# martinmodrak/math

Measured on AMD Instinct MI355X. Metric: gradient evals/sec (fp64), GP-marginal log-density N=4096, higher is better.
Workload: dtype f64; 1 GPU; gp_marginal_gradient; N=4096, kernel=exp_quad, parallelism=replicas1

## Files before the change

include/smg_hip.h:

```cpp
#ifndef SMG_HIP_H
#define SMG_HIP_H

#include <stddef.h>

#ifdef __cplusplus
extern "C" {
#endif

enum smg_status_code {
  SMG_OK = 0,
  SMG_ERR_HIP = 1,
  SMG_ERR_NOT_PD = 2,
  SMG_ERR_NOT_SYMMETRIC = 4,
  SMG_ERR_NONFINITE = 8,
  SMG_ERR_ARG = 16,
  SMG_ERR_OOM = 32,
  SMG_ERR_NOT_POSITIVE = 64,
  SMG_ERR_SYNC = 128
};

typedef struct smg_ctx smg_ctx;

int smg_device_count(int* n_host);
int smg_ctx_create(int device, size_t initial_arena_bytes, smg_ctx** out_host);
// ... 10 lines not shown
void* smg_host_scratch(smg_ctx* ctx, size_t bytes);
void* smg_pinned_io(smg_ctx* ctx, size_t bytes);
void* smg_pinned_result(smg_ctx* ctx, size_t bytes);
int smg_publish_to_host(smg_ctx* ctx, const double* src, long long n, double* dst);
int smg_gather_scalars(smg_ctx* ctx, const double* const* src, int n, double* dst, int* status_out);

int smg_memcpy_h2d(smg_ctx* ctx, void* dst, const void* src_host, size_t bytes);
int smg_memcpy_d2h(smg_ctx* ctx, void* dst_host, const void* src, size_t bytes);
int smg_memcpy_d2d(smg_ctx* ctx, void* dst, const void* src, size_t bytes);
int smg_memset(smg_ctx* ctx, void* dst, int value, size_t bytes);
int smg_memset_async(smg_ctx* ctx, void* dst, size_t bytes);
int smg_join_async(smg_ctx* ctx);
int smg_sync(smg_ctx* ctx);
int smg_sync_all(smg_ctx* ctx);
int smg_marker_record(smg_ctx* ctx, int slot);
int smg_marker_wait(smg_ctx* ctx, int slot);
int smg_status(smg_ctx* ctx, int* status_host);
int smg_status_armed(smg_ctx* ctx, int* armed);
int smg_status_enqueue(smg_ctx* ctx, int* host_dst);
int smg_status_inject(smg_ctx* ctx, int bits);
int smg_set_inv_block_mode(smg_ctx* ctx, int mode);
int smg_inv_block_fused(smg_ctx* ctx, int n);
int smg_set_gemm_stage_mode(smg_ctx* ctx, int mode);

enum smg_family {
  SMG_FAM_GEMM = 0, SMG_FAM_CHOL_FWD = 1, SMG_FAM_CHOL_REV = 2,
  SMG_FAM_GP = 3, SMG_FAM_MVN = 4, SMG_FAM_TRSV = 5, SMG_FAM_GLM = 6,
  SMG_FAM_ELEMWISE = 7,
  SMG_FAM_PANEL = 8,
  SMG_FAM_COMM = 9,
  SMG_FAM_COUNT = 10
};
int smg_profile_enable(smg_ctx* ctx, int on);
int smg_profile_read(smg_ctx* ctx, int family, double* total_ms_host, long long* count_host);
int smg_profile_flops(smg_ctx* ctx, int family, double* flops_host);

int smg_fill_unif(smg_ctx* ctx, double* out, long long n, unsigned long long seed,
                  double a, double b, double scale);
int smg_fill_bernoulli(smg_ctx* ctx, int* out, long long n, unsigned long long seed, double p);

int smg_gemm(smg_ctx* ctx, int transA, int transB, int uplo, int m, int n, int k,
             double alpha, const double* A, int lda, const double* B, int ldb,
             double beta, double* C, int ldc);
#define SMG_TRI_A_LOWER 1
#define SMG_TRI_A_UPPER 2
#define SMG_TRI_B_LOWER 4
#define SMG_TRI_B_UPPER 8
int smg_gemm_tri(smg_ctx* ctx, int transA, int transB, int uplo, int tri, int m, int n, int k, double alpha,
                 const double* A, int lda, const double* B, int ldb, double beta, double* C, int ldc);
int smg_gemm_bz(smg_ctx* ctx, int transA, int transB, int uplo, int tri, int m, int n, int k, double alpha,
                const double* A, int lda, const double* B, int ldb, double beta, double* C, int ldc, int bz);


int smg_gp_exp_quad_cov_fwd(smg_ctx* ctx, const double* x, int n, double sigma,
                            double l, double* K, int ldk);
int smg_gp_exp_quad_cov_rev(smg_ctx* ctx, const double* x, int n, double sigma,
                            double l, const double* Kadj, int ldka, double* out2);

int smg_gp_exp_quad_cov_nd_fwd(smg_ctx* ctx, const double* x, int D, int n, double sigma,
                               double l, double* K, int ldk);
int smg_gp_exp_quad_cov_nd_rev(smg_ctx* ctx, const double* x, int D, int n, double sigma,
                               double l, const double* Kadj, int ldka, double* out2);

enum smg_gp_family { SMG_GP_EXP_QUAD = 0, SMG_GP_EXPONENTIAL = 1, SMG_GP_MATERN32 = 2, SMG_GP_MATERN52 = 3 };
int smg_gp_cov_fwd(smg_ctx* ctx, int family, const double* x, int D, int n, double sigma, double l,
                   double* K, int ldk);
int smg_gp_cov_rev(smg_ctx* ctx, int family, const double* x, int D, int n, double sigma, double l,
                   const double* Kadj, int ldka, double* out2);

int smg_gp_exp_quad_cov_tangent_fwd(smg_ctx* ctx, const double* x, int n, double sigma,
                                    double l, double dsigma, double dl, double* Kd, int ldk);
int smg_gp_exp_quad_cov_tangent_rev(smg_ctx* ctx, const double* x, int n, double sigma,
                                    double l, double dsigma, double dl, const double* Kdadj,
                                    int ldka, double* out4);
// ... 246 lines not shown
```

math_amd/csrc/chol_mvn.hip:

```cpp
#include "smg_internal.h"
#include "tri_small.h"
#include "gp_family.h"

#include <vector>

namespace {

int inv_t_rec(smg_ctx* ctx, const double* L, int ldl, const double* w512, int n, double* V, int ldv, double* T,
              int lo, int hi, bool pairs) {
  if (hi - lo == SMG_NBR || (pairs && hi - lo == 2 * SMG_NBR)) return SMG_OK;
  const int mid = lo + ((hi - lo) / SMG_NBR / 2) * SMG_NBR;
  int rc = inv_t_rec(ctx, L, ldl, w512, n, V, ldv, T, lo, mid, pairs);
  if (!rc) rc = inv_t_rec(ctx, L, ldl, w512, n, V, ldv, T, mid, hi, pairs);
  if (rc) return rc;
  const int b = mid - lo, a = hi - mid;
  rc = smg_gemm_impl(ctx, 0, 1, 0, b, a, b, 1.0, V + lo + (size_t)lo * ldv, ldv, L + mid + (size_t)lo * ldl, ldl, 0.0,
                     T, n, SMG_TRI_A_UPPER);
  if (rc) return rc;
  return smg_gemm_impl(ctx, 0, 0, 0, b, a, a, -1.0, T, n, V + mid + (size_t)mid * ldv, ldv, 0.0,
                       V + lo + (size_t)mid * ldv, ldv, SMG_TRI_B_UPPER);
}

__global__ __launch_bounds__(256) void k_leaf_transpose(const double* __restrict__ w512, int n, int lo,
                                                       double* __restrict__ V, int ldv) {
// ... 294 lines not shown
  else if (pairs)
    hipLaunchKernelGGL((k_gp_inv_reduce<F, true, true>), dim3(nb), dim3(256), 0, ctx->stream, C, ldc, n, s, k,
                       s_stride, K0, ldk, x, D, cl, s2, part);
  else
    hipLaunchKernelGGL((k_gp_inv_reduce<F, false, true>), dim3(nb), dim3(256), 0, ctx->stream, C, ldc, n, s, k,
                       s_stride, K0, ldk, x, D, cl, s2, part);
  hipLaunchKernelGGL(k_gp_inv_final<F>, dim3(1), dim3(1024), 0, ctx->stream, part, nb, adj, sigma, l, dadj, out2);
  SMG_LAUNCH_CHECK();
  return SMG_OK;
}

}

bool smg_inv_prog_ok(int n) { return n % SMG_NBR == 0 && n >= 2 * SMG_NBR; }

int smg_inv_prog_init(smg_ctx* ctx, int n, double* ws) {
  (void)ctx;
  (void)n;
  (void)ws;
  return SMG_OK;
}

static int prog_acc(smg_ctx* ctx, int ta, int uplo, int m, int nc, int kk, const double* A, int lda,
                    const double* B, int ldb, double* C, int ldc, int bz, bool first) {
  if (first) return smg_gemm_impl(ctx, ta, 0, uplo, m, nc, kk, 1.0, A, lda, B, ldb, 0.0, C, ldc);
  return smg_gemm_bz_impl(ctx, ta, 0, uplo, m, nc, kk, 1.0, A, lda, B, ldb, 1.0, C, ldc, 0, bz);
}

int smg_inv_prog_row(smg_ctx* ctx, const double* L, int ldl, double* aux, int n, double* ws, int k, int part,
                     bool inverses_here) {
  constexpr int P = SMG_NBR;
  const size_t nn = (size_t)n * n;
  double* W = ws;
  double* C = ws + nn;
  double* Y = C + nn;
  double* T = Y + nn;
  const int r0 = k * P, r1 = r0 + P;
  const double* Wkk = aux + (size_t)n * SMG_AUX_W512 + r0;
  int rc;
  switch (part) {
    case 0:
      if (inverses_here) {
        bool wrote = false;
        if ((rc = smg_block_inverses_rows(ctx, L, ldl, aux, n, r0, P, T, W + r0 + (size_t)r0 * n, &wrote)))
          return rc;
        SMG_HIP_TRY(hipEventRecord(ctx->inv_ev_aux, ctx->stream));
        if (wrote) return SMG_OK;
      }
      return smg_copy_impl(ctx, P, P, Wkk, n, W + r0 + (size_t)r0 * n, n, 1.0, 0);
    case 1:
      if (k == 0) return SMG_OK;
      return smg_gemm_impl(ctx, 0, 0, 0, P, r0, P, -1.0, Wkk, n, Y + r0, n, 0.0, W + r0, n, SMG_TRI_A_LOWER);
    case 2:
      return prog_acc(ctx, 1, 1, r1, r1, P, W + r0, n, W + r0, n, C, n, r0, k == 0);
    case 3:
      if (r1 >= n) return SMG_OK;
      return prog_acc(ctx, 0, 0, P, r1, P, L + r1 + (size_t)r0 * ldl, ldl, W + r0, n, Y + r1, n, -r0, k == 0);
    default:
      if (r1 + P >= n) return SMG_OK;
      return prog_acc(ctx, 0, 0, n - r1 - P, r1, P, L + r1 + P + (size_t)r0 * ldl, ldl, W + r0, n, Y + r1 + P, n, -r0,
                      k == 0);
  }
}

double smg_inv_prog_cost(int n, int k, int part, bool inverses_here) {
  constexpr double P = SMG_NBR, rate = 30e6;
  const double r0 = k * P, r1 = r0 + P;
  switch (part) {
    case 0: return inverses_here ? 60.0 : 6.0;
    case 1: return k == 0 ? 0.0 : 6.0 + P * r0 * P / rate;
    case 2: return 6.0 + r1 * r1 * P / rate;
    case 3: return r1 >= n ? 0.0 : 6.0 + 2.0 * P * r1 * P / rate;
    default: return r1 + P >= n ? 0.0 : 6.0 + 2.0 * (n - r1 - P) * r1 * P / rate;
  }
}

extern "C" {

size_t smg_cholesky_mvn_rev_ws_doubles(int n) {
  return n > 0 ? 3 * (size_t)n * n + SMG_NBR / 2 * 256 : 0;
}

int smg_cholesky_mvn_rev(smg_ctx* ctx, const double* L, int ldl, const double* aux, int n, const double* s, int k,
                         long long s_stride, double adj, double* Aadj, int ldaa, double* ws) {
  if (!ctx || n < 0 || k < 1 || (k > 1 && s_stride < n)) return SMG_ERR_ARG;
  if (n == 0) return SMG_OK;
  if (!L || !ws || ldl < n || (Aadj && (!s || ldaa < n))) return SMG_ERR_ARG;
  smg_prof_scope prof(ctx, SMG_FAM_CHOL_REV);
  const size_t nn = (size_t)n * n;
  double* V = ws;
  double* C = ws + nn;
  int rc;
  if (v_by_doubling(n, aux)) {
    if ((rc = form_v(ctx, L, ldl, aux, n, V, C))) return rc;
    rc = smg_gemm_impl(ctx, 0, 1, 1, n, n, n, 1.0, V, n, V, n, 0.0, C, n, SMG_TRI_A_UPPER | SMG_TRI_B_LOWER);
  } else {
// ... 165 lines not shown
```

math_amd/csrc/cholesky.hip:

```cpp
#include <chrono>
#include "smg_internal.h"
#include "tri_small.h"
#include "smg_sync.h"
#include <cstdlib>
#include <vector>

namespace {

__global__ __launch_bounds__(256) void k_check_symmetric(const double* __restrict__ A, int lda,
                                                         int n, int* status) {
  __shared__ double T[64][65];
  int bi, bj;
  {
    const int t = blockIdx.x;
    int r = (int)((sqrt(8.0 * (double)t + 1.0) - 1.0) * 0.5);
    while ((r + 1) * (r + 2) / 2 <= t) ++r;
    while (r * (r + 1) / 2 > t) --r;
    bi = r;
    bj = t - r * (r + 1) / 2;
  }
  const int i0 = 64 * bi, j0 = 64 * bj;
  const int lane = threadIdx.x & 63, w = threadIdx.x >> 6;
  for (int c = w; c < 64; c += 4) {
    const int gr = j0 + lane, gc = i0 + c;
    T[c][lane] = (gr < n && gc < n) ? A[gr + (size_t)gc * lda] : 0.0;
  }
  __syncthreads();
  bool bad = false;
// ... 1621 lines not shown
        smg_on_side on(ctx);
        rc = smg_gemm_impl(ctx, 0, 1, 1, m2, K3 - K2, K - J, -1.0, P2, ldl, P2, ldl, 1.0,
                           L + K2 + (size_t)K2 * ldl, ldl);
      }
      if (rc) return rc;
      F = smg_event(ctx, nev++);
      if (!F) return SMG_ERR_HIP;
      SMG_HIP_TRY(hipEventRecord(F, ctx->side));
      if (K3 < n) {
        const int m3 = n - K3;
        const double* P3 = L + K3 + (size_t)J * ldl;
        smg_on_side on(ctx);
        if ((rc = smg_gemm_impl(ctx, 0, 1, 1, m3, m3, K - J, -1.0, P3, ldl, P3, ldl, 1.0, L + K3 + (size_t)K3 * ldl,
                                ldl)))
          return rc;
      }
    } else if (prog) {
      SMG_HIP_TRY(hipStreamWaitEvent(ctx->side, E, 0));
    }
    if (prog) {
      const double m2 = n - K2, kk = K - J;
      const double slack = 22.0 * (K2 - K) / SMG_NB + 6.0 + (double)(n - K) * (K2 - K) * kk / 30e6 -
                           (K2 < n ? 6.0 + m2 * m2 * kk / 40e6 : 0.0);
      if ((rc = queue_parts(J / NB2, 0.5 * slack))) return rc;
    }
  }
  if (prog) {
    if (int rc0 = queue_parts(rows_prog - 2, -1.0)) return rc0;
  }
  if (mark) {
    const int rc = smg_status_mark_impl(ctx);
    if (rc) return rc;
  }
  if (F) SMG_HIP_TRY(hipStreamWaitEvent(ctx->stream, F, 0));
  int rc;
  if (prog) {
    const int r0 = n - SMG_NBR;
    SMG_HIP_TRY(hipStreamWaitEvent(ctx->stream, ctx->inv_ev_aux, 0));
    bool wkk = false;
    if ((rc = chol_block_inverses(ctx, L, ldl, aux, n, r0, SMG_NBR, nullptr, true, inv_ws + r0 + (size_t)r0 * n,
                                  &wkk)))
      return rc;
    SMG_HIP_TRY(hipEventRecord(ctx->inv_ev_main, ctx->stream));
    const int klast = n / SMG_NBR - 1;
    if (zero_parts) {
      SMG_HIP_TRY(hipStreamWaitEvent(ctx->zero_stream, ctx->inv_ev_main, 0));
      hipStream_t keep = ctx->stream;
// ... 67 lines not shown
```

math_amd/csrc/ctx.hip:

```cpp
#include <cstdio>
#include <cstdlib>
#include <cstring>

#include "smg_internal.h"

namespace {

constexpr size_t kAlign = 256;

__global__ void k_reduce_partials(const double* __restrict__ p, int nparts,
                                  int width, double* out, int accumulate) {
  __shared__ double lds[16];
  const int c = blockIdx.x;
  double s = 0.0;
  for (int i = threadIdx.x; i < nparts; i += blockDim.x) s += p[(size_t)i * width + c];
  s = block_sum(s, lds);
  if (threadIdx.x == 0) out[c] = accumulate ? out[c] + s : s;
}

__global__ __launch_bounds__(256) void k_publish(const double* __restrict__ src, long long n, double* dst,
                                                 long long* done, long long seq) {
  for (long long i = threadIdx.x; i < n; i += blockDim.x)
    __hip_atomic_store(dst + i, src[i], __ATOMIC_RELAXED, __HIP_MEMORY_SCOPE_SYSTEM);
  asm volatile("s_waitcnt vmcnt(0)" ::: "memory");
// ... 209 lines not shown
    return SMG_ERR_HIP;
  }
  if (initial < (size_t)(64u << 20)) initial = (size_t)(64u << 20);
  char* base = nullptr;
  if (hipMalloc(&base, initial) != hipSuccess) {
    hipStreamDestroy(ctx->stream);
    delete ctx;
    return SMG_ERR_OOM;
  }
  ctx->blocks.push_back({base, initial});
  if (hipMalloc(&ctx->status_d, SMG_STATUS_BYTES) != hipSuccess ||
      hipHostMalloc(&ctx->status_h, 256, hipHostMallocDefault) != hipSuccess) {
    delete ctx;
    return SMG_ERR_HIP;
  }
  hipMemset(ctx->status_d, 0, SMG_STATUS_BYTES);
  ctx->flags_d = ctx->status_d + 64;
  ctx->flag_epoch = 0;
  ctx->inv_ctr_d = reinterpret_cast<unsigned*>(ctx->flags_d + 4096);
  ctx->inv_launches = 0;
  ctx->inv_per_cu = ctx->inv_cus = -1;
  ctx->inv_mode = 0;
  ctx->gemm_stage = 0;
  ctx->host_scratch_size = 1u << 20;
  if (hipHostMalloc(&ctx->host_scratch, ctx->host_scratch_size, hipHostMallocDefault) != hipSuccess) {
    delete ctx;
    return SMG_ERR_HIP;
  }
  if (hipHostMalloc(&ctx->done_h, 256, hipHostMallocCoherent | hipHostMallocMapped) != hipSuccess ||
      hipMalloc(&ctx->red_counter_d, 256) != hipSuccess) {
    delete ctx;
    return SMG_ERR_HIP;
  }
  *(volatile long long*)ctx->done_h = 0;
  hipMemset(ctx->red_counter_d, 0, 256);
  hipDeviceSynchronize();
  *out = ctx;
  return SMG_OK;
}

int smg_ctx_destroy(smg_ctx* ctx) {
  if (!ctx) return SMG_OK;
  hipSetDevice(ctx->device);
  hipStreamSynchronize(ctx->stream);
  prof_drain(ctx);
  smg_comm_destroy(ctx);
// ... 350 lines not shown
  if (int rc = smg_marker_event(ctx, slot, &e)) return rc;
  SMG_HIP_TRY(hipEventRecord(e, ctx->stream));
  return SMG_OK;
}

int smg_marker_wait(smg_ctx* ctx, int slot) {
  if (!ctx || slot < 0 || slot >= (int)ctx->marker_ev.size()) return SMG_ERR_ARG;
  SMG_HIP_TRY(hipEventSynchronize(ctx->marker_ev[slot]));
  return SMG_OK;
}

int smg_set_inv_block_mode(smg_ctx* ctx, int mode) {
  if (!ctx || mode < 0 || mode > 1) return SMG_ERR_ARG;
  ctx->inv_mode = mode;
  return SMG_OK;
}

int smg_set_gemm_stage_mode(smg_ctx* ctx, int mode) {
  if (!ctx || mode < 0 || mode > 2) return SMG_ERR_ARG;
  ctx->gemm_stage = mode;
  return SMG_OK;
}

int smg_sync_all(smg_ctx* ctx) {
  if (!ctx) return SMG_ERR_ARG;
  sync_all_streams(ctx);
  SMG_HIP_TRY(hipGetLastError());
  if (ctx->prof_on) prof_drain(ctx);
  return SMG_OK;
}

int smg_sync(smg_ctx* ctx) {
  SMG_HIP_TRY(hipStreamSynchronize(ctx->stream));
  if (ctx->prof_on) prof_drain(ctx);
  return SMG_OK;
}

int smg_status(smg_ctx* ctx, int* status) {
  hipLaunchKernelGGL(k_status_take, dim3(1), dim3(64), 0, ctx->stream, ctx->status_d, ctx->status_h);
  SMG_LAUNCH_CHECK();
  SMG_HIP_TRY(hipStreamSynchronize(ctx->stream));
  if (ctx->prof_on) prof_drain(ctx);
  int s = ctx->status_h[0] | ctx->host_status;
  ctx->host_status = 0;
  ctx->status_armed = 0;
  if (status) *status = s;
// ... 137 lines not shown
```

math_amd/csrc/gemm.hip:

```cpp
#include "smg_internal.h"
#include <cstdio>
#include <cstdlib>
#include <type_traits>

#ifndef SMG_GEMM_TRI128_MIN
#define SMG_GEMM_TRI128_MIN 1024
#endif
#ifndef SMG_GEMM_KS2_MAX
#define SMG_GEMM_KS2_MAX 1536
#endif
#ifndef SMG_GEMM_DMA_BK1
#define SMG_GEMM_DMA_BK1 16
#endif
#ifndef SMG_GEMM_DMA_NB1
#define SMG_GEMM_DMA_NB1 3
#endif
#ifndef SMG_GEMM_DMA_BK2
#define SMG_GEMM_DMA_BK2 32
#endif
#ifndef SMG_GEMM_DMA_NB2
#define SMG_GEMM_DMA_NB2 2
#endif
#ifndef SMG_GEMM_DMA_KS2_MAX
#define SMG_GEMM_DMA_KS2_MAX 512
// ... 122 lines not shown
  tri_decode(t, r, c);
  const int r0 = r / G * G, r1 = min(r0 + G, T), h = r1 - r0;
  int q = t - r0 * (r0 + 1) / 2;
  if (q < r0 * h) {
    bi = r0 + q % h;
    bj = q / h;
    return;
  }
  q -= r0 * h;
  int j = r0;
  while (q >= r1 - j) {
    q -= r1 - j;
    ++j;
  }
  bi = j + q;
  bj = j;
}

template <int BM, int BN, int BK, bool TA, bool TB, int MODE, int KS = 1, int NB = 0>
__global__ __launch_bounds__(256 * KS) void k_gemm(
    int m, int n, int k, double alpha, const double* __restrict__ A, int lda,
    const double* __restrict__ B, int ldb, double beta, double* __restrict__ C,
    int ldc, int tiles_m, int ntiles, int kchunk, double* __restrict__ slab, long long sA,
    long long sB, long long sC, int px, int ntp, int tri, double* __restrict__ C2, int ldc2, int bz) {
  constexpr bool LOWT = MODE == 1 || MODE == 3;
  constexpr bool UPT = MODE == 2;
  constexpr bool TRIC = LOWT || UPT;
  A += blockIdx.y * sA;
  B += blockIdx.y * sB;
  C += blockIdx.y * sC;
  constexpr bool AK = TA;
  constexpr bool BKC = !TB;
  using LA = lds_layout<BM, BK, AK>;
  using LB = lds_layout<BN, BK, BKC>;
  constexpr int NR = BM == 128 ? 1 : (BM == 64 ? SMG_GEMM_NR64 : SMG_GEMM_NR32);
  constexpr int STAGE = LA::size + LB::size;
  constexpr int OPS = (NB ? NB : 2) * STAGE;
  constexpr int ECH = (BM * BN + BN <= OPS) ? BN : 32;
  constexpr int POOL = (OPS > (BM + 1) * ECH) ? OPS : (BM + 1) * ECH;
  __shared__ double pool[POOL];

  int bi, bj, tile, split;
  const bool tri_a_only = !TRIC && (tri & 3) && !(tri & 12);
  const bool tri_b_only = !TRIC && (tri & 12) && !(tri & 3);
  if (px > 0) {
    split = blockIdx.x / ntp;
    const int tb = blockIdx.x - split * ntp;
    const int x = tb & 7, l = tb >> 3, py = 8 / px;
    const int tiles_n = ntiles / tiles_m;
    const int rx = x % px, ry = x / px;
    const int r0 = rx * tiles_m / px, r1 = (rx + 1) * tiles_m / px;
    const int c0 = ry * tiles_n / py, c1 = (ry + 1) * tiles_n / py;
    const int rm = r1 - r0;
    if (rm <= 0 || l >= rm * (c1 - c0)) return;
    tile = (r0 + l % rm) + (c0 + l / rm) * tiles_m;
  } else {
    tile = blockIdx.x % ntiles;
    split = blockIdx.x / ntiles;
  }
  const bool tri_sq = TRIC && m == n && BM == BN;
  if (LOWT && tri_sq) {
    const int T = tiles_m;
    int r, q;
    if (tri == SMG_TRI_B_LOWER) {
      tri_decode(ntiles - 1 - tile, r, q);
      bj = T - 1 - r;
      bi = bj + q;
    } else if (tri == SMG_TRI_B_UPPER || tri == (SMG_TRI_A_LOWER | SMG_TRI_B_UPPER)) {
      tri_decode(tile, r, q);
      bj = T - 1 - r;
      bi = bj + q;
    } else if (tri == (SMG_TRI_A_LOWER | SMG_TRI_B_LOWER)) {
      tri_decode(tile, r, q);
      bj = q;
      bi = q + (T - 1 - r);
    } else if (tri == SMG_TRI_A_LOWER) {
      tri_decode(ntiles - 1 - tile, bi, bj);
    } else if (tri == 0 && ntiles >= 64) {
      const int b = tile, x = b & 7, per = ntiles >> 3, extra = ntiles & 7;
      tri_decode_grouped(x * per + (x < extra ? x : extra) + (b >> 3), tiles_m, bi, bj);
    } else {
      tri_decode(tile, bi, bj);
    }
  } else if (UPT && tri_sq) {
    tri_decode(tile, bj, bi);
  } else if (tri_a_only) {
    const int r = tile / (ntiles / tiles_m);
    bi = (tri & 1) ? tiles_m - 1 - r : r;
    bj = tile % (ntiles / tiles_m);
  } else if (tri_b_only) {
    const int tn = ntiles / tiles_m, c = tile / tiles_m;
    bi = tile % tiles_m;
    bj = (tri & 8) ? tn - 1 - c : c;
  } else {
    bi = tile % tiles_m;
    bj = tile / tiles_m;
  }
  if (LOWT && !tri_sq && bj * BN > bi * BM + BM - 1) return;
  if (UPT && !tri_sq && bi * BM > bj * BN + BN - 1) return;
  const int i0 = bi * BM, j0 = bj * BN;
  int kbeg = split * kchunk;
  int kend = min(k, kbeg + kchunk);
  if (tri) {
    int lo = 0, hi = k;
    if (tri & 1) hi = min(hi, i0 + BM);
    if (tri & 2) lo = max(lo, i0);
    if (tri & 4) lo = max(lo, j0);
    if (tri & 8) hi = min(hi, j0 + BN);
    lo = lo / BK * BK;
    kbeg = max(kbeg, lo);
    kend = min(kend, hi);
    if (kend < kbeg) kend = kbeg;
  }

  constexpr int TM = BM / 32, TN = BN / 32;
  constexpr int NT = 256 * KS;
  const int lane = threadIdx.x & 63, wave = threadIdx.x >> 6;
  const int wr = (wave & 3) >> 1, wc = wave & 1, kg = KS == 1 ? 0 : wave >> 2;
  d4 acc[TM][TN];
#pragma unroll
  for (int a = 0; a < TM; ++a)
#pragma unroll
    for (int b = 0; b < TN; ++b) acc[a][b] = d4{0.0, 0.0, 0.0, 0.0};

  constexpr int PA = BM * BK / NT, PB = BN * BK / NT;
  double ra[NR][PA], rb[NR][PB];
  const int nst = (kend - kbeg + BK - 1) / BK;
  auto gload = [&](int set, int st) {
    load_tile<BM, BK, AK, NT>(A, lda, m, kend, i0, kbeg + st * BK, ra[set]);
    load_tile<BN, BK, BKC, NT>(B, ldb, n, kend, j0, kbeg + st * BK, rb[set]);
  };
// ... 187 lines not shown
    int t = 0;
    for (; t + 4 <= splits; t += 4) {
      const d2v a0 = *reinterpret_cast<const d2v*>(slab + (size_t)t * tot + e);
      const d2v a1 = *reinterpret_cast<const d2v*>(slab + (size_t)(t + 1) * tot + e);
      const d2v a2 = *reinterpret_cast<const d2v*>(slab + (size_t)(t + 2) * tot + e);
      const d2v a3 = *reinterpret_cast<const d2v*>(slab + (size_t)(t + 3) * tot + e);
      s += a0;
      s += a1;
      s += a2;
      s += a3;
    }
    for (; t < splits; ++t) s += *reinterpret_cast<const d2v*>(slab + (size_t)t * tot + e);
    double* c = C + i + (size_t)j * ldc;
    const bool w0 = !(lower == 1 && i < j), w1 = !(lower == 2 && i + 1 > j);
    const double b = ((bz > 0 && i >= bz) || (bz < 0 && j >= -bz)) ? 0.0 : beta;
    if (w0) c[0] = (b == 0.0) ? alpha * s[0] : alpha * s[0] + b * c[0];
    if (w1) c[1] = (b == 0.0) ? alpha * s[1] : alpha * s[1] + b * c[1];
  }
}

thread_local double* t_c2 = nullptr;
thread_local int t_ldc2 = 0;
thread_local int t_bz = 0;

template <int BM, int BN, int BK, bool TA, bool TB, int MODE, int KS = 1, int NB = 0>
int launch(smg_ctx* ctx, int m, int n, int k, double alpha, const double* A,
           int lda, const double* B, int ldb, double beta, double* C, int ldc, int batch = 1,
           long long sA = 0, long long sB = 0, long long sC = 0, int tri = 0) {
  constexpr bool TRIC = MODE == 1 || MODE == 2 || MODE == 3;
  const int tm = smg_ceil_div(m, BM), tn = smg_ceil_div(n, BN);
  const int ntiles = (TRIC && m == n && BM == BN) ? tm * (tm + 1) / 2 : tm * tn;
  int splits = 1;
  const int target = 512;
  constexpr int KMIN = 64;
  const bool covers = ntiles >= 256 && k <= 1024;
  if (NB == 0 && !tri && MODE != 3 && MODE != 4 && batch == 1 && ntiles < target && !covers &&
      k >= 2 * KMIN) {
    splits = smg_ceil_div(target, ntiles);
    const int maxs = k / KMIN;
    if (splits > maxs) splits = maxs;
    if (splits > 64) splits = 64;
    if (splits < 1) splits = 1;
  }
  int kchunk = smg_ceil_div(smg_ceil_div(k, splits), BK) * BK;
  splits = smg_ceil_div(k, kchunk);
  double* slab = nullptr;
  if (splits > 1) {
    const int slot = ctx->stream == ctx->side                                ? SMG_WS_GEMM_SIDE
                     : (ctx->zero_stream && ctx->stream == ctx->zero_stream) ? SMG_WS_GEMM_ZERO
                                                                             : SMG_WS_GEMM;
    slab = smg_ws(ctx, slot, (size_t)splits * m * n);
    if (!slab) return SMG_ERR_OOM;
  }
  const bool tri_one = !TRIC && tri && (!(tri & 3) || !(tri & 12));
  int px = 0, ntp = ntiles;
  if (!(TRIC && m == n && BM == BN) && ntiles >= 64 && !tri_one) {
    long long best = -1;
    for (int p = 1; p <= 8; p *= 2) {
      const int q = 8 / p;
      if (p > tm || q > tn) continue;
      const long long rr = smg_ceil_div(tm, p), cc = smg_ceil_div(tn, q);
      const long long foot = rr * BM + cc * BN;
      if (best < 0 || foot < best) {
        best = foot;
        px = p;
        ntp = 8 * (int)(rr * cc);
      }
    }
  }
  hipLaunchKernelGGL((k_gemm<BM, BN, BK, TA, TB, MODE, KS, NB>), dim3(ntp * splits, batch), dim3(256 * KS), 0,
                     ctx->stream, m, n, k, alpha, A, lda, B, ldb, beta, C, ldc, tm,
                     ntiles, kchunk, slab, sA, sB, sC, px, ntp, tri, MODE >= 3 ? t_c2 : nullptr,
                     MODE >= 3 ? t_ldc2 : 0, t_bz);
  if (splits > 1) {
    const long long tot = (long long)m * n;
    if ((m & 1) == 0) {
      const long long pairs = tot / 2;
      const int nb = (int)(pairs / 256 < 2048 ? (pairs + 255) / 256 : 2048);
      hipLaunchKernelGGL(k_splitk_reduce2, dim3(nb), dim3(256), 0, ctx->stream, m, n, splits, slab, alpha, beta,
                         C, ldc, MODE, t_bz);
    } else {
      hipLaunchKernelGGL(k_splitk_reduce, dim3(smg_ceil_div(tot, 256)), dim3(256), 0,
                         ctx->stream, m, n, splits, slab, alpha, beta, C, ldc, MODE, t_bz);
    }
  }
  SMG_LAUNCH_CHECK();
  return SMG_OK;
}

inline bool overlaps(const double* X, int ldx, int rows, int cols, const double* C, int ldc, int m,
                     int n) {
  if (rows <= 0 || cols <= 0 || m <= 0 || n <= 0) return false;
  const double* x1 = X + (size_t)(cols - 1) * ldx + rows;
  const double* c1 = C + (size_t)(n - 1) * ldc + m;
  if (!(X < c1 && C < x1)) return false;
  if (ldx != ldc) return true;
// ... 116 lines not shown
    if (!ta && !tb) return dispatch_tile<false, false, 1>(ctx, m, n, k, alpha, A, lda, B, ldb, beta, C, ldc, tri);
    return dispatch_tile<true, true, 1>(ctx, m, n, k, alpha, A, lda, B, ldb, beta, C, ldc, tri);
  }
  if (uplo == 3) {
    if (ta && !tb) return dispatch_tile<true, false, 3>(ctx, m, n, k, alpha, A, lda, B, ldb, beta, C, ldc, tri);
    if (!ta && !tb) return dispatch_tile<false, false, 3>(ctx, m, n, k, alpha, A, lda, B, ldb, beta, C, ldc, tri);
    if (!ta && tb) return dispatch_tile<false, true, 3>(ctx, m, n, k, alpha, A, lda, B, ldb, beta, C, ldc, tri);
    return dispatch_tile<true, true, 3>(ctx, m, n, k, alpha, A, lda, B, ldb, beta, C, ldc, tri);
  }
  if (uplo == 2) {
    if (!ta && tb) return dispatch_tile<false, true, 2>(ctx, m, n, k, alpha, A, lda, B, ldb, beta, C, ldc, tri);
    if (ta && !tb) return dispatch_tile<true, false, 2>(ctx, m, n, k, alpha, A, lda, B, ldb, beta, C, ldc, tri);
    if (!ta && !tb) return dispatch_tile<false, false, 2>(ctx, m, n, k, alpha, A, lda, B, ldb, beta, C, ldc, tri);
    return dispatch_tile<true, true, 2>(ctx, m, n, k, alpha, A, lda, B, ldb, beta, C, ldc, tri);
  }
  if (!ta && !tb) return dispatch_tile<false, false, 0>(ctx, m, n, k, alpha, A, lda, B, ldb, beta, C, ldc, tri);
  if (!ta && tb) return dispatch_tile<false, true, 0>(ctx, m, n, k, alpha, A, lda, B, ldb, beta, C, ldc, tri);
  if (ta && !tb) return dispatch_tile<true, false, 0>(ctx, m, n, k, alpha, A, lda, B, ldb, beta, C, ldc, tri);
  return dispatch_tile<true, true, 0>(ctx, m, n, k, alpha, A, lda, B, ldb, beta, C, ldc, tri);
}

int smg_gemm_bz_impl(smg_ctx* ctx, int ta, int tb, int uplo, int m, int n, int k, double alpha, const double* A,
                     int lda, const double* B, int ldb, double beta, double* C, int ldc, int tri, int bz) {
  if (bz % 128) return SMG_ERR_ARG;
  t_bz = bz;
  const int rc = smg_gemm_impl(ctx, ta, tb, uplo, m, n, k, alpha, A, lda, B, ldb, beta, C, ldc, tri);
  t_bz = 0;
  return rc;
}

int smg_gemm_dual_impl(smg_ctx* ctx, int ta, int tb, int m, int n, int k, double alpha, const double* A, int lda,
                       const double* B, int ldb, double beta, double* C, int ldc, double* C2, int ldc2, int tri) {
  if (m <= 0 || n <= 0) return SMG_OK;
  if (k <= 0 || alpha == 0.0 || !C2) return SMG_ERR_ARG;
  smg_prof_scope prof(ctx, SMG_FAM_GEMM);
  if (ctx->prof_on) ctx->prof_flops[SMG_FAM_GEMM] += 2.0 * m * n * k;
  t_c2 = C2;
  t_ldc2 = ldc2;
  int rc;
  if (!ta && !tb) rc = dispatch_tile<false, false, 4>(ctx, m, n, k, alpha, A, lda, B, ldb, beta, C, ldc, tri);
  else if (ta && !tb) rc = dispatch_tile<true, false, 4>(ctx, m, n, k, alpha, A, lda, B, ldb, beta, C, ldc, tri);
  else if (!ta && tb) rc = dispatch_tile<false, true, 4>(ctx, m, n, k, alpha, A, lda, B, ldb, beta, C, ldc, tri);
  else rc = dispatch_tile<true, true, 4>(ctx, m, n, k, alpha, A, lda, B, ldb, beta, C, ldc, tri);
  t_c2 = nullptr;
  return rc;
}

int smg_gemm_sym_phi_impl(smg_ctx* ctx, int ta, int tb, int n, int k, double alpha, const double* A, int lda,
                          const double* B, int ldb, double beta, double* C, int ldc, double* P, int ldp, int tri) {
  if (n <= 0) return SMG_OK;
// ... 14 lines not shown
  return rc;
}

extern "C" int smg_gemm_tri(smg_ctx* ctx, int ta, int tb, int uplo, int tri, int m, int n, int k,
                            double alpha, const double* A, int lda, const double* B, int ldb, double beta,
                            double* C, int ldc) {
  if (!ctx || m < 0 || n < 0 || k < 0 || tri < 0 || tri > 15) return SMG_ERR_ARG;
  if ((m > 0 && n > 0) && (!C || ldc < m)) return SMG_ERR_ARG;
  if (k > 0 && m > 0 && n > 0 && alpha != 0.0) {
    if (!A || !B) return SMG_ERR_ARG;
    if (lda < (ta ? k : m) || ldb < (tb ? n : k)) return SMG_ERR_ARG;
  }
  return smg_gemm_impl(ctx, ta, tb, uplo, m, n, k, alpha, A, lda, B, ldb, beta, C, ldc, tri);
}

extern "C" int smg_gemm_bz(smg_ctx* ctx, int ta, int tb, int uplo, int tri, int m, int n, int k, double alpha,
                           const double* A, int lda, const double* B, int ldb, double beta, double* C, int ldc,
                           int bz) {
  if (!ctx || m <= 0 || n <= 0 || k <= 0 || tri < 0 || tri > 15 || alpha == 0.0) return SMG_ERR_ARG;
  if (!A || !B || !C || ldc < m || lda < (ta ? k : m) || ldb < (tb ? n : k)) return SMG_ERR_ARG;
  return smg_gemm_bz_impl(ctx, ta, tb, uplo, m, n, k, alpha, A, lda, B, ldb, beta, C, ldc, tri, bz);
}

extern "C" int smg_gemm(smg_ctx* ctx, int ta, int tb, int uplo, int m, int n, int k,
                        double alpha, const double* A, int lda, const double* B,
                        int ldb, double beta, double* C, int ldc) {
  if (!ctx || m < 0 || n < 0 || k < 0) return SMG_ERR_ARG;
  if ((m > 0 && n > 0) && (!C || ldc < m)) return SMG_ERR_ARG;
  if (k > 0 && m > 0 && n > 0 && alpha != 0.0) {
    if (!A || !B) return SMG_ERR_ARG;
    if (lda < (ta ? k : m) || ldb < (tb ? n : k)) return SMG_ERR_ARG;
  }
  return smg_gemm_impl(ctx, ta, tb, uplo, m, n, k, alpha, A, lda, B, ldb, beta, C, ldc);
}
```

math_amd/csrc/smg_internal.h:

```cpp
#pragma once
#include <hip/hip_runtime.h>

#include <cstddef>
#include <cstdint>
#include <utility>
#include <vector>

#include "../../include/smg_hip.h"

typedef double d4 __attribute__((ext_vector_type(4)));
typedef double d2v __attribute__((ext_vector_type(2)));

struct smg_arena_block {
  char* base;
  size_t size;
};

struct smg_prof_slot {
  hipEvent_t start, stop;
  int family;
};

constexpr int SMG_INV_CTRS = 64;
constexpr size_t SMG_STATUS_BYTES = 256 + 4096 * sizeof(int) + SMG_INV_CTRS * sizeof(int);

struct smg_ctx {
  int device;
  hipStream_t stream;
  hipStream_t side;
  hipStream_t main_stream;
  std::vector<hipEvent_t> ev_pool;
// ... 4 lines not shown
  size_t offset;
  int* status_d;
  int* status_h;
  int host_status;
  int status_armed;
  hipEvent_t status_ev;
  int status_mark;
  hipStream_t zero_stream;
  hipStream_t copy_stream;
  hipEvent_t zero_ev_main, zero_ev_done;
  int zero_pending;
  std::vector<std::pair<void*, size_t>> zero_queue;
  hipEvent_t inv_ev, inv_ev_main, inv_ev_aux;
  int inv_pending;
  hipEvent_t inv_ev_w;
  int inv_w_recorded;
  int* flags_d;
  int flag_epoch;
  unsigned* inv_ctr_d;
  long long inv_launches;
  int inv_per_cu, inv_cus;
  int inv_mode;
  int gemm_stage;
  void* host_scratch;
  size_t host_scratch_size;
  void* pin_io;
  size_t pin_io_size;
  void* res_h;
  size_t res_h_size;
  long long* done_h;
  long long done_seq;
  unsigned int* red_counter_d;
  double* ws[12];
  size_t ws_doubles[12];
  int prof_on;
  std::vector<smg_prof_slot> prof_pending;
  std::vector<hipEvent_t> prof_pool;
  double prof_ms[SMG_FAM_COUNT];
  double prof_flops[SMG_FAM_COUNT];
  long long prof_count[SMG_FAM_COUNT];
  void* comm;
};

#define SMG_HIP_TRY(expr)                          \
  do {                                             \
    hipError_t _e = (expr);                        \
// ... 60 lines not shown
                  const double* aux = nullptr);
extern "C" int smg_add_sym_from_upper(smg_ctx* ctx, int n, const double* S, int lds, double* B, int ldb);
int smg_copy_impl(smg_ctx* ctx, int m, int n, const double* A, int lda, double* B, int ldb,
                  double alpha, int accumulate);
int smg_status_mark_impl(smg_ctx* ctx);
int smg_zero_ranges_impl(smg_ctx* ctx, hipStream_t stream, const std::pair<void*, size_t>* r, int count,
                         unsigned max_grid = 2048);
extern "C" int smg_d2h_impl(smg_ctx* ctx, hipStream_t stream, void* dst, const void* src, size_t bytes);
extern "C" int smg_zero_flush(smg_ctx* ctx);
extern "C" int smg_zero_stream_begin(smg_ctx* ctx);
extern "C" int smg_marker_event(smg_ctx* ctx, int slot, hipEvent_t* ev);
extern "C" int smg_pack_tril_cols(smg_ctx* ctx, int n, const double* A, int lda, int j0, int j1, double* dst);
int smg_trtri_blocks_impl(smg_ctx* ctx, const double* L, int ldl, int n, double* W);
int smg_block_inverses_impl(smg_ctx* ctx, const double* L, int ldl, double* aux, int n);
int smg_trsv_lower_impl(smg_ctx* ctx, int trans, const double* L, int ldl, const double* W64,
                        const double* W256, const double* W512, int ldw, const double* x, double* y,
                        double* r, int n);

int smg_gemm_impl(smg_ctx* ctx, int transA, int transB, int uplo, int m, int n,
                  int k, double alpha, const double* A, int lda, const double* B,
                  int ldb, double beta, double* C, int ldc, int tri = 0);
int smg_gemm_bz_impl(smg_ctx* ctx, int ta, int tb, int uplo, int m, int n, int k, double alpha, const double* A,
                     int lda, const double* B, int ldb, double beta, double* C, int ldc, int tri, int bz);

int smg_gemm_dual_impl(smg_ctx* ctx, int ta, int tb, int m, int n, int k, double alpha, const double* A, int lda,
                       const double* B, int ldb, double beta, double* C, int ldc, double* C2, int ldc2,
                       int tri = 0);

int smg_gemm_sym_phi_impl(smg_ctx* ctx, int ta, int tb, int n, int k, double alpha, const double* A, int lda,
                          const double* B, int ldb, double beta, double* C, int ldc, double* P, int ldp, int tri);

int smg_gemm_batched_impl(smg_ctx* ctx, int ta, int tb, int m, int n, int k, double alpha,
                          const double* A, int lda, long long sA, const double* B, int ldb,
                          long long sB, double beta, double* C, int ldc, long long sC, int batch);

void smg_reduce_partials(smg_ctx* ctx, const double* partials, int nparts,
                         int width, double* out, int accumulate);

static inline int smg_ceil_div(long long a, long long b) { return (int)((a + b - 1) / b); }

__device__ __forceinline__ double wave_sum(double v) {
#pragma unroll
  for (int off = 32; off > 0; off >>= 1) v += __shfl_xor(v, off, 64);
  return v;
}
__device__ __forceinline__ double wave_max(double v) {
// ... 42 lines not shown
```

math_amd/hip.py:

```python
import ctypes
import os

import numpy as np

_HERE = os.path.dirname(os.path.abspath(__file__))
LIB_PATH = os.path.join(_HERE, "lib", "libsmg_hip.so")

SMG_OK = 0
STATUS = {1: "hip", 2: "not_pd", 4: "not_symmetric", 8: "nonfinite", 16: "arg", 32: "oom", 64: "not_positive"}
GP_FAMILIES = {"exp_quad": 0, "exponential": 1, "matern32": 2, "matern52": 3}
FAMILIES = {"gemm": 0, "chol_fwd": 1, "chol_rev": 2, "gp": 3, "mvn": 4, "trsv": 5, "glm": 6, "elementwise": 7, "panel": 8, "comm": 9}

_P = ctypes.c_void_p
_I = ctypes.c_int
_L = ctypes.c_longlong
_D = ctypes.c_double
_S = ctypes.c_size_t

_SIGS = {
    "smg_device_count": (_I, [ctypes.POINTER(_I)]),
    "smg_ctx_create": (_I, [_I, _S, ctypes.POINTER(_P)]),
    "smg_ctx_destroy": (_I, [_P]),
    "smg_ctx_device": (_I, [_P]),
    "smg_ctx_stream": (_P, [_P]),
    "smg_arena_alloc": (_P, [_P, _S]),
    "smg_arena_mark": (_S, [_P]),
    "smg_arena_rewind": (_I, [_P, _S]),
    "smg_arena_recover_all": (_I, [_P]),
    "smg_arena_used": (_S, [_P]),
    "smg_arena_reserved": (_S, [_P]),
    "smg_host_scratch": (_P, [_P, _S]),
    "smg_memcpy_h2d": (_I, [_P, _P, _P, _S]),
    "smg_memcpy_d2h": (_I, [_P, _P, _P, _S]),
    "smg_memcpy_d2d": (_I, [_P, _P, _P, _S]),
    "smg_memset": (_I, [_P, _P, _I, _S]),
    "smg_memset_async": (_I, [_P, _P, _S]),
    "smg_join_async": (_I, [_P]),
    "smg_sync": (_I, [_P]),
    "smg_sync_all": (_I, [_P]),
    "smg_status": (_I, [_P, ctypes.POINTER(_I)]),
    "smg_status_armed": (_I, [_P, ctypes.POINTER(_I)]),
    "smg_status_enqueue": (_I, [_P, _P]),
    "smg_status_inject": (_I, [_P, _I]),
    "smg_set_inv_block_mode": (_I, [_P, _I]),
    "smg_inv_block_fused": (_I, [_P, _I]),
    "smg_set_gemm_stage_mode": (_I, [_P, _I]),
    "smg_pinned_io": (_P, [_P, _S]),
    "smg_pinned_result": (_P, [_P, _S]),
    "smg_gather_scalars": (_I, [_P, _P, _I, _P, _P]),
    "smg_pack_tril": (_I, [_P, _I, _I, _P, _I, _P]),
    "smg_unpack_tril_add": (_I, [_P, _I, _I, _P, _P, _I]),
    "smg_publish_to_host": (_I, [_P, _P, _L, _P]),
    "smg_profile_enable": (_I, [_P, _I]),
    "smg_profile_read": (_I, [_P, _I, ctypes.POINTER(_D), ctypes.POINTER(_L)]),
    "smg_profile_flops": (_I, [_P, _I, ctypes.POINTER(_D)]),
    "smg_fill_unif": (_I, [_P, _P, _L, ctypes.c_ulonglong, _D, _D, _D]),
    "smg_fill_bernoulli": (_I, [_P, _P, _L, ctypes.c_ulonglong, _D]),
    "smg_gemm": (_I, [_P, _I, _I, _I, _I, _I, _I, _D, _P, _I, _P, _I, _D, _P, _I]),
    "smg_gemm_tri": (_I, [_P, _I, _I, _I, _I, _I, _I, _I, _D, _P, _I, _P, _I, _D, _P, _I]),
    "smg_gemm_bz": (_I, [_P, _I, _I, _I, _I, _I, _I, _I, _D, _P, _I, _P, _I, _D, _P, _I, _I]),
    "smg_gp_exp_quad_cov_fwd": (_I, [_P, _P, _I, _D, _D, _P, _I]),
    "smg_gp_exp_quad_cov_rev": (_I, [_P, _P, _I, _D, _D, _P, _I, _P]),
    "smg_bernoulli_logit_glm_checked": (_I, [_P, _P, _P, _L, _I, _L, _P, _P, _P]),
    "smg_bernoulli_logit_glm_io": (_I, [_P, _P, _P, _L, _I, _L, _D, _P, _P, _P, _P]),
    "smg_marker_record": (_I, [_P, _I]),
    "smg_marker_wait": (_I, [_P, _I]),
    "smg_gp_exp_quad_cov_nd_fwd": (_I, [_P, _P, _I, _I, _D, _D, _P, _I]),
    "smg_gp_exp_quad_cov_nd_rev": (_I, [_P, _P, _I, _I, _D, _D, _P, _I, _P]),
    "smg_add_diag_fwd": (_I, [_P, _P, _I, _I, _D, _P, _P, _I]),
    "smg_add_diag_rev": (_I, [_P, _P, _I, _I, _P, _I, _P, _I]),
    "smg_cholesky_block_size": (_I, [_I]),
    "smg_check_symmetric": (_I, [_P, _P, _I, _I]),
    "smg_cholesky_fwd": (_I, [_P, _P, _I, _I, _P, _I, _P]),
    "smg_cholesky_fwd_checked": (_I, [_P, _P, _I, _I, _P, _I, _P]),
    "smg_cholesky_fwd_checked_mark": (_I, [_P, _P, _I, _I, _P, _I, _P]),
    "smg_status_mark_wait": (_I, [_P, _P]),
    "smg_cholesky_rev": (_I, [_P, _P, _I, _P, _P, _I, _I, _P, _I]),
    "smg_mdivide_left_tri_fwd": (_I, [_P, _I, _P, _I, _P, _I, _I, _I, _P, _I]),
    "smg_mdivide_left_tri_rev": (_I, [_P, _I, _P, _I, _P, _I, _P, _I, _I, _I, _P, _I, _P, _I, _P]),
    "smg_mdivide_left_tri_aux_fwd": (_I, [_P, _I, _P, _I, _P, _P, _I, _I, _I, _P, _I]),
    "smg_mdivide_left_tri_aux_rev": (_I, [_P, _I, _P, _I, _P, _P, _I, _P, _I, _I, _I, _P, _I, _P, _I, _P]),
    "smg_chol_tangent_fwd": (_I, [_P, _P, _I, _P, _P, _I, _I, _P, _P, _P, _P, _P, _I]),
    "smg_chol_tangent_fwd_w": (_I, [_P, _P, _I, _P, _P, _I, _I, _P, _P, _P, _P, _I]),
# ... 209 lines not shown
```

Before: 456.1 gradient evals/s.

## Skip structurally-zero K ranges in progressive inverse GEMMs via per-tile cuts

Adds cut_a/cut_b parameters to the GEMM kernel so each tile raises its lower K bound where the progressive block-inverse operands are known to be zero (triangular structure of W rows). It also redistributes tiles (dealing columns across partitions and grouping uncut tiles) to balance the now-uneven per-tile work, and updates the cost model used for scheduling. This cuts wasted FLOPs in the inverse accumulation GEMMs, at the price of more kernel indexing logic and a reliance on the zero-structure assumption holding.

```diff
diff --git a/include/smg_hip.h b/include/smg_hip.h
--- a/include/smg_hip.h
+++ b/include/smg_hip.h
@@ -56,6 +56,7 @@
 int smg_set_inv_block_mode(smg_ctx* ctx, int mode);
 int smg_inv_block_fused(smg_ctx* ctx, int n);
 int smg_set_gemm_stage_mode(smg_ctx* ctx, int mode);
+int smg_set_gemm_cut_mode(smg_ctx* ctx, int mode);
 
 enum smg_family {
   SMG_FAM_GEMM = 0, SMG_FAM_CHOL_FWD = 1, SMG_FAM_CHOL_REV = 2,
@@ -84,6 +85,9 @@
                  const double* A, int lda, const double* B, int ldb, double beta, double* C, int ldc);
 int smg_gemm_bz(smg_ctx* ctx, int transA, int transB, int uplo, int tri, int m, int n, int k, double alpha,
                 const double* A, int lda, const double* B, int ldb, double beta, double* C, int ldc, int bz);
+int smg_gemm_cut(smg_ctx* ctx, int transA, int transB, int uplo, int tri, int m, int n, int k, double alpha,
+                 const double* A, int lda, const double* B, int ldb, double beta, double* C, int ldc, int bz,
+                 int cut_a, int cut_b);
 
 
 int smg_gp_exp_quad_cov_fwd(smg_ctx* ctx, const double* x, int n, double sigma,
diff --git a/math_amd/csrc/chol_mvn.hip b/math_amd/csrc/chol_mvn.hip
--- a/math_amd/csrc/chol_mvn.hip
+++ b/math_amd/csrc/chol_mvn.hip
@@ -340,9 +340,9 @@
 }
 
 static int prog_acc(smg_ctx* ctx, int ta, int uplo, int m, int nc, int kk, const double* A, int lda,
-                    const double* B, int ldb, double* C, int ldc, int bz, bool first) {
-  if (first) return smg_gemm_impl(ctx, ta, 0, uplo, m, nc, kk, 1.0, A, lda, B, ldb, 0.0, C, ldc);
-  return smg_gemm_bz_impl(ctx, ta, 0, uplo, m, nc, kk, 1.0, A, lda, B, ldb, 1.0, C, ldc, 0, bz);
+                    const double* B, int ldb, double* C, int ldc, int bz, bool first, int cut_a, int cut_b) {
+  return smg_gemm_cut_impl(ctx, ta, 0, uplo, m, nc, kk, 1.0, A, lda, B, ldb, first ? 0.0 : 1.0, C, ldc, 0,
+                           first ? 0 : bz, cut_a, cut_b);
 }
 
 int smg_inv_prog_row(smg_ctx* ctx, const double* L, int ldl, double* aux, int n, double* ws, int k, int part,
@@ -370,26 +370,29 @@
       if (k == 0) return SMG_OK;
       return smg_gemm_impl(ctx, 0, 0, 0, P, r0, P, -1.0, Wkk, n, Y + r0, n, 0.0, W + r0, n, SMG_TRI_A_LOWER);
     case 2:
-      return prog_acc(ctx, 1, 1, r1, r1, P, W + r0, n, W + r0, n, C, n, r0, k == 0);
+      return prog_acc(ctx, 1, 1, r1, r1, P, W + r0, n, W + r0, n, C, n, r0, k == 0, r0, -1);
     case 3:
       if (r1 >= n) return SMG_OK;
-      return prog_acc(ctx, 0, 0, P, r1, P, L + r1 + (size_t)r0 * ldl, ldl, W + r0, n, Y + r1, n, -r0, k == 0);
+      return prog_acc(ctx, 0, 0, P, r1, P, L + r1 + (size_t)r0 * ldl, ldl, W + r0, n, Y + r1, n, -r0, k == 0, -1, r0);
     default:
       if (r1 + P >= n) return SMG_OK;
       return prog_acc(ctx, 0, 0, n - r1 - P, r1, P, L + r1 + P + (size_t)r0 * ldl, ldl, W + r0, n, Y + r1 + P, n, -r0,
-                      k == 0);
+                      k == 0, -1, r0);
   }
 }
 
 double smg_inv_prog_cost(int n, int k, int part, bool inverses_here) {
   constexpr double P = SMG_NBR, rate = 30e6;
+  constexpr double T = 64.0, ycut = P * (P - T);
   const double r0 = k * P, r1 = r0 + P;
+  double scut = 0.0;
+  for (int q = 1; q < SMG_NBR / 64; ++q) scut += 2.0 * T * (T * q) * (r0 + T * (q + 1));
   switch (part) {
     case 0: return inverses_here ? 60.0 : 6.0;
     case 1: return k == 0 ? 0.0 : 6.0 + P * r0 * P / rate;
-    case 2: return 6.0 + r1 * r1 * P / rate;
-    case 3: return r1 >= n ? 0.0 : 6.0 + 2.0 * P * r1 * P / rate;
-    default: return r1 + P >= n ? 0.0 : 6.0 + 2.0 * (n - r1 - P) * r1 * P / rate;
+    case 2: return 6.0 + (r1 * r1 * P - scut) / rate;
+    case 3: return r1 >= n ? 0.0 : 6.0 + (2.0 * P * r1 * P - P * ycut) / rate;
+    default: return r1 + P >= n ? 0.0 : 6.0 + (n - r1 - P) * (2.0 * r1 * P - ycut) / rate;
   }
 }
 
diff --git a/math_amd/csrc/cholesky.hip b/math_amd/csrc/cholesky.hip
--- a/math_amd/csrc/cholesky.hip
+++ b/math_amd/csrc/cholesky.hip
@@ -4,6 +4,10 @@
 #include "smg_sync.h"
 #include <cstdlib>
 #include <vector>
+
+#ifndef SMG_PROG_SLACK_SCALE
+#define SMG_PROG_SLACK_SCALE 0.5
+#endif
 
 namespace {
 
@@ -1671,7 +1675,7 @@
       const double m2 = n - K2, kk = K - J;
       const double slack = 22.0 * (K2 - K) / SMG_NB + 6.0 + (double)(n - K) * (K2 - K) * kk / 30e6 -
                            (K2 < n ? 6.0 + m2 * m2 * kk / 40e6 : 0.0);
-      if ((rc = queue_parts(J / NB2, 0.5 * slack))) return rc;
+      if ((rc = queue_parts(J / NB2, SMG_PROG_SLACK_SCALE * slack))) return rc;
     }
   }
   if (prog) {
diff --git a/math_amd/csrc/ctx.hip b/math_amd/csrc/ctx.hip
--- a/math_amd/csrc/ctx.hip
+++ b/math_amd/csrc/ctx.hip
@@ -255,6 +255,7 @@
   ctx->inv_per_cu = ctx->inv_cus = -1;
   ctx->inv_mode = 0;
   ctx->gemm_stage = 0;
+  ctx->gemm_cut = SMG_GEMM_CUT_DEFAULT;
   ctx->host_scratch_size = 1u << 20;
   if (hipHostMalloc(&ctx->host_scratch, ctx->host_scratch_size, hipHostMallocDefault) != hipSuccess) {
     delete ctx;
@@ -651,6 +652,12 @@
   return SMG_OK;
 }
 
+int smg_set_gemm_cut_mode(smg_ctx* ctx, int mode) {
+  if (!ctx || mode < 0 || mode > 2) return SMG_ERR_ARG;
+  ctx->gemm_cut = mode;
+  return SMG_OK;
+}
+
 int smg_sync_all(smg_ctx* ctx) {
   if (!ctx) return SMG_ERR_ARG;
   sync_all_streams(ctx);
diff --git a/math_amd/csrc/gemm.hip b/math_amd/csrc/gemm.hip
--- a/math_amd/csrc/gemm.hip
+++ b/math_amd/csrc/gemm.hip
@@ -168,7 +168,8 @@
     int m, int n, int k, double alpha, const double* __restrict__ A, int lda,
     const double* __restrict__ B, int ldb, double beta, double* __restrict__ C,
     int ldc, int tiles_m, int ntiles, int kchunk, double* __restrict__ slab, long long sA,
-    long long sB, long long sC, int px, int ntp, int tri, double* __restrict__ C2, int ldc2, int bz) {
+    long long sB, long long sC, int px, int ntp, int tri, double* __restrict__ C2, int ldc2, int bz, int cut_a,
+    int cut_b, int cut_spread) {
   constexpr bool LOWT = MODE == 1 || MODE == 3;
   constexpr bool UPT = MODE == 2;
   constexpr bool TRIC = LOWT || UPT;
@@ -198,8 +199,10 @@
     const int r0 = rx * tiles_m / px, r1 = (rx + 1) * tiles_m / px;
     const int c0 = ry * tiles_n / py, c1 = (ry + 1) * tiles_n / py;
     const int rm = r1 - r0;
-    if (rm <= 0 || l >= rm * (c1 - c0)) return;
-    tile = (r0 + l % rm) + (c0 + l / rm) * tiles_m;
+    const bool deal = cut_spread && cut_b >= 0;
+    const int nc = deal ? (tiles_n - ry + py - 1) / py : c1 - c0;
+    if (rm <= 0 || l >= rm * nc) return;
+    tile = (r0 + l % rm) + (deal ? ry + py * (l / rm) : c0 + l / rm) * tiles_m;
   } else {
     tile = blockIdx.x % ntiles;
     split = blockIdx.x / ntiles;
@@ -223,8 +226,15 @@
     } else if (tri == SMG_TRI_A_LOWER) {
       tri_decode(ntiles - 1 - tile, bi, bj);
     } else if (tri == 0 && ntiles >= 64) {
-      const int b = tile, x = b & 7, per = ntiles >> 3, extra = ntiles & 7;
-      tri_decode_grouped(x * per + (x < extra ? x : extra) + (b >> 3), tiles_m, bi, bj);
+      const int b = tile, x = b & 7, l = b >> 3;
+      int nu = 0;
+      if (cut_spread && cut_a >= 0) {
+        const int g0 = min((cut_a + BM - 1) / BM, T) / 8 * 8;
+        nu = (g0 * (g0 + 1) / 2) & ~7;
+      }
+      const int rest = ntiles - nu, per = rest >> 3, extra = rest & 7;
+      const int t = l < (nu >> 3) ? x * (nu >> 3) + l : nu + x * per + (x < extra ? x : extra) + l - (nu >> 3);
+      tri_decode_grouped(t, tiles_m, bi, bj);
     } else {
       tri_decode(tile, bi, bj);
     }
@@ -247,12 +257,14 @@
   const int i0 = bi * BM, j0 = bj * BN;
   int kbeg = split * kchunk;
   int kend = min(k, kbeg + kchunk);
-  if (tri) {
+  if (tri || cut_a >= 0 || cut_b >= 0) {
     int lo = 0, hi = k;
     if (tri & 1) hi = min(hi, i0 + BM);
     if (tri & 2) lo = max(lo, i0);
     if (tri & 4) lo = max(lo, j0);
     if (tri & 8) hi = min(hi, j0 + BN);
+    if (cut_a >= 0 && i0 >= cut_a) lo = max(lo, i0 - cut_a);
+    if (cut_b >= 0 && j0 >= cut_b) lo = max(lo, j0 - cut_b);
     lo = lo / BK * BK;
     kbeg = max(kbeg, lo);
     kend = min(kend, hi);
@@ -486,6 +498,30 @@
 thread_local double* t_c2 = nullptr;
 thread_local int t_ldc2 = 0;
 thread_local int t_bz = 0;
+thread_local int t_cut_a = -1, t_cut_b = -1;
+
+template <int BM, int BN, int BK>
+double cut_flops(int mode, int m, int n, int k, int cut_a, int cut_b) {
+  double f = 0.0;
+  for (int j0 = 0; j0 < n; j0 += BN)
+    for (int i0 = 0; i0 < m; i0 += BM) {
+      int lo = 0;
+      if (cut_a >= 0 && i0 >= cut_a) lo = i0 - cut_a;
+      if (cut_b >= 0 && j0 >= cut_b && j0 - cut_b > lo) lo = j0 - cut_b;
+      lo = lo / BK * BK;
+      if (lo > k) lo = k;
+      if (lo == 0) continue;
+      const int i1 = i0 + BM < m ? i0 + BM : m, j1 = j0 + BN < n ? j0 + BN : n;
+      double el = 0.0;
+      for (int j = j0; j < j1; ++j) {
+        const int a = (mode == 1 || mode == 3) && j > i0 ? j : i0;
+        const int b = mode == 2 && j + 1 < i1 ? j + 1 : i1;
+        if (b > a) el += b - a;
+      }
+      f += 2.0 * lo * el;
+    }
+  return f;
+}
 
 template <int BM, int BN, int BK, bool TA, bool TB, int MODE, int KS = 1, int NB = 0>
 int launch(smg_ctx* ctx, int m, int n, int k, double alpha, const double* A,
@@ -494,6 +530,10 @@
   constexpr bool TRIC = MODE == 1 || MODE == 2 || MODE == 3;
   const int tm = smg_ceil_div(m, BM), tn = smg_ceil_div(n, BN);
   const int ntiles = (TRIC && m == n && BM == BN) ? tm * (tm + 1) / 2 : tm * tn;
+  const int cut_a = ctx->gemm_cut ? t_cut_a : -1, cut_b = ctx->gemm_cut ? t_cut_b : -1;
+  const int cut_spread = ctx->gemm_cut == 1;
+  if (ctx->prof_on && !tri && (cut_a >= 0 || cut_b >= 0))
+    ctx->prof_flops[SMG_FAM_GEMM] -= batch * cut_flops<BM, BN, BK>(MODE, m, n, k, cut_a, cut_b);
   int splits = 1;
   const int target = 512;
   constexpr int KMIN = 64;
@@ -535,7 +575,7 @@
   hipLaunchKernelGGL((k_gemm<BM, BN, BK, TA, TB, MODE, KS, NB>), dim3(ntp * splits, batch), dim3(256 * KS), 0,
                      ctx->stream, m, n, k, alpha, A, lda, B, ldb, beta, C, ldc, tm,
                      ntiles, kchunk, slab, sA, sB, sC, px, ntp, tri, MODE >= 3 ? t_c2 : nullptr,
-                     MODE >= 3 ? t_ldc2 : 0, t_bz);
+                     MODE >= 3 ? t_ldc2 : 0, t_bz, cut_a, cut_b, cut_spread);
   if (splits > 1) {
     const long long tot = (long long)m * n;
     if ((m & 1) == 0) {
@@ -698,10 +738,19 @@
 
 int smg_gemm_bz_impl(smg_ctx* ctx, int ta, int tb, int uplo, int m, int n, int k, double alpha, const double* A,
                      int lda, const double* B, int ldb, double beta, double* C, int ldc, int tri, int bz) {
-  if (bz % 128) return SMG_ERR_ARG;
+  return smg_gemm_cut_impl(ctx, ta, tb, uplo, m, n, k, alpha, A, lda, B, ldb, beta, C, ldc, tri, bz, -1, -1);
+}
+
+int smg_gemm_cut_impl(smg_ctx* ctx, int ta, int tb, int uplo, int m, int n, int k, double alpha, const double* A,
+                      int lda, const double* B, int ldb, double beta, double* C, int ldc, int tri, int bz, int cut_a,
+                      int cut_b) {
+  if (bz % 128 || cut_a < -1 || cut_b < -1) return SMG_ERR_ARG;
   t_bz = bz;
+  t_cut_a = cut_a;
+  t_cut_b = cut_b;
   const int rc = smg_gemm_impl(ctx, ta, tb, uplo, m, n, k, alpha, A, lda, B, ldb, beta, C, ldc, tri);
   t_bz = 0;
+  t_cut_a = t_cut_b = -1;
   return rc;
 }
 
@@ -762,6 +811,14 @@
   return smg_gemm_bz_impl(ctx, ta, tb, uplo, m, n, k, alpha, A, lda, B, ldb, beta, C, ldc, tri, bz);
 }
 
+extern "C" int smg_gemm_cut(smg_ctx* ctx, int ta, int tb, int uplo, int tri, int m, int n, int k, double alpha,
+                            const double* A, int lda, const double* B, int ldb, double beta, double* C, int ldc,
+                            int bz, int cut_a, int cut_b) {
+  if (!ctx || m <= 0 || n <= 0 || k <= 0 || tri < 0 || tri > 15 || alpha == 0.0) return SMG_ERR_ARG;
+  if (!A || !B || !C || ldc < m || lda < (ta ? k : m) || ldb < (tb ? n : k)) return SMG_ERR_ARG;
+  return smg_gemm_cut_impl(ctx, ta, tb, uplo, m, n, k, alpha, A, lda, B, ldb, beta, C, ldc, tri, bz, cut_a, cut_b);
+}
+
 extern "C" int smg_gemm(smg_ctx* ctx, int ta, int tb, int uplo, int m, int n, int k,
                         double alpha, const double* A, int lda, const double* B,
                         int ldb, double beta, double* C, int ldc) {
diff --git a/math_amd/csrc/smg_internal.h b/math_amd/csrc/smg_internal.h
--- a/math_amd/csrc/smg_internal.h
+++ b/math_amd/csrc/smg_internal.h
@@ -7,6 +7,10 @@
 #include <vector>
 
 #include "../../include/smg_hip.h"
+
+#ifndef SMG_GEMM_CUT_DEFAULT
+#define SMG_GEMM_CUT_DEFAULT 1
+#endif
 
 typedef double d4 __attribute__((ext_vector_type(4)));
 typedef double d2v __attribute__((ext_vector_type(2)));
@@ -57,6 +61,7 @@
   int inv_per_cu, inv_cus;
   int inv_mode;
   int gemm_stage;
+  int gemm_cut;
   void* host_scratch;
   size_t host_scratch_size;
   void* pin_io;
@@ -163,6 +168,9 @@
                   int ldb, double beta, double* C, int ldc, int tri = 0);
 int smg_gemm_bz_impl(smg_ctx* ctx, int ta, int tb, int uplo, int m, int n, int k, double alpha, const double* A,
                      int lda, const double* B, int ldb, double beta, double* C, int ldc, int tri, int bz);
+int smg_gemm_cut_impl(smg_ctx* ctx, int ta, int tb, int uplo, int m, int n, int k, double alpha, const double* A,
+                      int lda, const double* B, int ldb, double beta, double* C, int ldc, int tri, int bz, int cut_a,
+                      int cut_b);
 
 int smg_gemm_dual_impl(smg_ctx* ctx, int ta, int tb, int m, int n, int k, double alpha, const double* A, int lda,
                        const double* B, int ldb, double beta, double* C, int ldc, double* C2, int ldc2,
diff --git a/math_amd/hip.py b/math_amd/hip.py
--- a/math_amd/hip.py
+++ b/math_amd/hip.py
@@ -45,6 +45,7 @@
     "smg_set_inv_block_mode": (_I, [_P, _I]),
     "smg_inv_block_fused": (_I, [_P, _I]),
     "smg_set_gemm_stage_mode": (_I, [_P, _I]),
+    "smg_set_gemm_cut_mode": (_I, [_P, _I]),
     "smg_pinned_io": (_P, [_P, _S]),
     "smg_pinned_result": (_P, [_P, _S]),
     "smg_gather_scalars": (_I, [_P, _P, _I, _P, _P]),
@@ -59,6 +60,7 @@
     "smg_gemm": (_I, [_P, _I, _I, _I, _I, _I, _I, _D, _P, _I, _P, _I, _D, _P, _I]),
     "smg_gemm_tri": (_I, [_P, _I, _I, _I, _I, _I, _I, _I, _D, _P, _I, _P, _I, _D, _P, _I]),
     "smg_gemm_bz": (_I, [_P, _I, _I, _I, _I, _I, _I, _I, _D, _P, _I, _P, _I, _D, _P, _I, _I]),
+    "smg_gemm_cut": (_I, [_P, _I, _I, _I, _I, _I, _I, _I, _D, _P, _I, _P, _I, _D, _P, _I, _I, _I, _I]),
     "smg_gp_exp_quad_cov_fwd": (_I, [_P, _P, _I, _D, _D, _P, _I]),
     "smg_gp_exp_quad_cov_rev": (_I, [_P, _P, _I, _D, _D, _P, _I, _P]),
     "smg_bernoulli_logit_glm_checked": (_I, [_P, _P, _P, _L, _I, _L, _P, _P, _P]),
```

New measurement: 470.9 gradient evals/s, median of 6. 3.3% higher.
